# puzzlepaint/surfelmeshing

Measured on NVIDIA H100. Metric: RGB-D frames/s at 640x480 (depth pre-processing + Integrate()), higher is better.
Workload: dtype f32

## Files before the change

surfelmeshing_b200/csrc/integrate.cu:

```cuda

#include <algorithm>
#include <cstdio>
#include <cstdlib>

#include <cooperative_groups.h>

#include "sm_kernels.cuh"

namespace cg = cooperative_groups;

namespace smb {

namespace {

#define SM_S(row, i) d.surfels[static_cast<size_t>(row) * d.stride + (i)]
#define SM_SU(row, i) reinterpret_cast<u32*>(d.surfels)[static_cast<size_t>(row) * d.stride + (i)]

constexpr int kBlock = 256;

__device__ __forceinline__ bool is_active(u32 last_update_stamp, u32 frame_index, int window) {
  return static_cast<int>(last_update_stamp) > static_cast<int>(frame_index - static_cast<u32>(window));
}

struct Projection {
// ... 35 lines not shown
__device__ __forceinline__ float normal_z_abs(float nx, float ny) {
  return fsqrt_approx(fmaxf(0.f, ffma(-ny, ny, ffma(-nx, nx, 1.0f))));
}

__device__ __forceinline__ float facing_dot(const FrameParams& f, float x, float y, float z, float nx, float ny,
                                            float nz, float3* local_normal) {
  const float rs = frsqrt_approx(squared_norm(x, y, z));
  *local_normal = rotate_vec(f.local_T_global, nx, ny, nz);
  return fmul(rs, ffma(z, local_normal->z, ffma(x, local_normal->x, fmul(y, local_normal->y))));
}

template <typename Body>
__device__ __forceinline__ void for_each_visible(const DeviceState& d, const u32* surfel_count, Body&& body) {
  constexpr u32 kItemsPerSegment = kSegment / kBlock;
  const u32 max_items = ((d.capacity + kSegment - 1) / kSegment) * kItemsPerSegment;
  const u32 n = *surfel_count;
  u32 item = blockIdx.x;
  u32 cnt = 0;
  VisEntry e = make_uint4(0u, 0u, 0u, 0u);
  if (item < max_items) {
    cnt = d.seg_count[item / kItemsPerSegment];
    e = d.vis[static_cast<size_t>(item) * kBlock + threadIdx.x];
  }
  const u32 items = ((n + kSegment - 1) / kSegment) * kItemsPerSegment;
  while (item < items) {
    const u32 next = item + gridDim.x;
    u32 cnt_next = 0;
    VisEntry e_next = e;
    if (next < items) {
      cnt_next = d.seg_count[next / kItemsPerSegment];
      e_next = d.vis[static_cast<size_t>(next) * kBlock + threadIdx.x];
    }
    const u32 k = (item % kItemsPerSegment) * kBlock + threadIdx.x;
    if (k < cnt) body(static_cast<size_t>(item) * kBlock + threadIdx.x, e);
    item = next;
    cnt = cnt_next;
    e = e_next;
  }
}

__global__ void __launch_bounds__(kBlock) k_clear(DeviceState d) {
  pdl_prologue();
  const int n = d.width * d.height;
  for (int i = blockIdx.x * blockDim.x + threadIdx.x; i < n; i += gridDim.x * blockDim.x) {
    d.assoc[i] = make_uint4(kInvalidIndex, kInvalidIndex, 0u, 0u);
    d.first_depth[i] = __int_as_float(0x7f800000);
    d.supported[i] = 0;
  }
}

constexpr int kProjectBlock = 512;

enum { kProjectAll = 0, kProjectMain = 1, kProjectTail = 2 };

__global__ void __launch_bounds__(kProjectBlock) k_project(DeviceState d, FrameParams f, int part) {
  pdl_prologue();
  if (f.skip) return;
  const TimelineScope timeline_scope(d, f.frame_index, part == kProjectTail ? KID_PROJECT_TAIL : KID_PROJECT);
  __shared__ u32 warp_totals[kProjectBlock / 32];
  const int lane = threadIdx.x & 31, warp = threadIdx.x >> 5;
  const u32 first_seg_if_all = blockIdx.x;

  if (blockIdx.x == 0 && part != kProjectMain) {
    const int tiles = (d.width * d.height + kSegment - 1) / kSegment;
    for (int t = threadIdx.x; t < tiles; t += blockDim.x) d.scan_state[t] = 0ull;
    if (threadIdx.x == 0) { d.counters->scan_ticket = 0; *d.upd_count = 0; }
  }

  struct SlotRows { float2 X, Y, Z; uint2 T; };
  auto fetch = [&](u32 seg) {
    SlotRows r;
    const size_t base = static_cast<size_t>(seg) * kSegment + threadIdx.x * 2;
    r.X = *reinterpret_cast<const float2*>(&SM_S(SM_ROW_X, base));
    r.Y = *reinterpret_cast<const float2*>(&SM_S(SM_ROW_Y, base));
    r.Z = *reinterpret_cast<const float2*>(&SM_S(SM_ROW_Z, base));
    r.T = *reinterpret_cast<const uint2*>(&SM_SU(SM_ROW_LAST_UPDATE_STAMP, base));
    return r;
  };
  SlotRows rows = {};
  if (part != kProjectTail && (static_cast<size_t>(first_seg_if_all) + 1) * kSegment <= d.stride) rows = fetch(first_seg_if_all);
  const u32 n_before = part == kProjectAll ? 0u : d.counters->surfel_count[(f.count_slot + kCountSlots - 1) % kCountSlots];
  const u32 seg_begin = part == kProjectTail ? n_before / kSegment : 0u;
  const u32 n = part == kProjectMain ? (n_before / kSegment) * kSegment
                                     : d.counters->surfel_count[f.count_slot];
  if (part == kProjectTail && static_cast<u64>(seg_begin + blockIdx.x) * kSegment < n) rows = fetch(seg_begin + blockIdx.x);
  for (u32 seg = seg_begin + blockIdx.x; static_cast<u64>(seg) * kSegment < n; seg += gridDim.x) {
    const u32 base = seg * kSegment + threadIdx.x * 2;
    const SlotRows cur = rows;
    if (static_cast<u64>(seg + gridDim.x) * kSegment < n) rows = fetch(seg + gridDim.x);
    VisEntry e[2];
    bool visible[2] = {false, false};
    u32 cnt = 0;
    if (base < n) {
      const float xs[2] = {cur.X.x, cur.X.y}, ys[2] = {cur.Y.x, cur.Y.y}, zs[2] = {cur.Z.x, cur.Z.y};
      const u32 ts[2] = {cur.T.x, cur.T.y};
#pragma unroll
      for (int j = 0; j < 2; ++j) {
        const u32 i = base + j;
        if (i >= n) break;
        const float z = transform_row(f.local_T_global.r2, xs[j], ys[j], zs[j]);
        if (!(z > 0.f)) continue;
        const float x = transform_row(f.local_T_global.r0, xs[j], ys[j], zs[j]);
        const float y = transform_row(f.local_T_global.r1, xs[j], ys[j], zs[j]);
        const Projection p = project(f, d.width, d.height, x, y, z);
        if (!p.in_image) continue;
        const bool active = is_active(ts[j], f.frame_index, f.active_window);
        e[j] = make_uint4(i | (active ? kActiveBit : 0u), __float_as_uint(x), __float_as_uint(y), __float_as_uint(z));
        visible[j] = true;
        ++cnt;
        if (active) {
          atomicMin(reinterpret_cast<int*>(&d.first_depth[p.py * d.width + p.px]), __float_as_int(z));
          int ox, oy;
          if (secondary_pixel(p, d.width, d.height, &ox, &oy)) {
            atomicMin(reinterpret_cast<int*>(&d.first_depth[oy * d.width + ox]), __float_as_int(z));
          }
        }
      }
    }
    u32 incl = cnt;
#pragma unroll
// ... 87 lines not shown
      if (!pass[k]) continue;
      const PixelGate& g = k == 0 ? g0 : g1;
      const int pp = k == 0 ? p.py * d.width + p.px : oy * d.width + ox;
      if (!(g.measurement_depth > 0.f)) { pass[k] = false; continue; }
      if (g.first < fmul(g.measurement_depth, fadd(-f.sensor_noise_factor, 1.0f))) {
        if (g.first == z) d.assoc[pp].y = idx;
        pass[k] = false;
        continue;
      }
      if (z > fmul(fadd(f.sensor_noise_factor, 1.0f), g.measurement_depth)) pass[k] = false;
    }
    if (!pass[0] && !pass[1]) return;
    const float snx = SM_S(SM_ROW_NORMAL_X, idx), sny = SM_S(SM_ROW_NORMAL_Y, idx), snz = SM_S(SM_ROW_NORMAL_Z, idx);
    const float surfel_radius_squared = SM_S(SM_ROW_RADIUS_SQUARED, idx);
    g0.normal = row_ptr(f.normals, f.normals_pitch, pass[0] ? p.py : oy)[pass[0] ? p.px : ox];
    g1.normal = row_ptr(f.normals, f.normals_pitch, pass[1] ? oy : p.py)[pass[1] ? ox : p.px];
    float3 ln;
    const float dot_angle = facing_dot(f, x, y, z, snx, sny, snz, &ln);
#endif
#pragma unroll
    for (int k = 0; k < 2; ++k) {
      if (!pass[k]) continue;
      const int pp = k == 0 ? p.py * d.width + p.px : oy * d.width + ox;
#if SM_ASSOCIATE_LEVELS == 1
      if (!supports_surfel(d, f, k == 0 ? g0 : g1, pp, idx, z, dot_angle, ln)) continue;
#else
      {
        const PixelGate& g = k == 0 ? g0 : g1;
        if (dot_angle > 0.f) continue;
        if (g.measurement_depth < z) {
          const float s = normal_z_abs(g.normal.x, g.normal.y);
          const float dot2 = ffma(-ln.z, s, ffma(ln.x, g.normal.x, fmul(ln.y, g.normal.y)));
          if (dot2 < f.cos_normal_compatibility_threshold) continue;
        }
      }
#endif
      if (!(surfel_radius_squared > 0.f)) continue;
      PixelAssoc* a = &d.assoc[pp];
      atomicMin(&a->x, tb_encode(f.tb, idx, k == 1, static_cast<u32>(pp)));
      atomicAdd(&a->z, 1u);
      atomicAdd(reinterpret_cast<float*>(&a->w), z);
      d.supported[pp] = 1;
    }
  });
}

#ifndef SM_MERGE_LEVELS
#define SM_MERGE_LEVELS 2
#endif
__global__ void __launch_bounds__(kBlock) k_merge(DeviceState d, FrameParams f) {
  pdl_prologue();
  if (f.skip) return;
  const TimelineScope timeline_scope(d, f.frame_index, KID_MERGE);
  u32 merged_by_thread = 0;
#if SM_MERGE_LEVELS == 2
  for_each_visible(d, &d.counters->surfel_count[f.count_slot], [&](size_t pos, const VisEntry& e) {
    const u32 idx = e.x & ~kActiveBit;
    const float x = __uint_as_float(e.y), y = __uint_as_float(e.z), z = __uint_as_float(e.w);
    const Projection p = project(f, d.width, d.height, x, y, z);
    const int pp = p.py * d.width + p.px;
    const float surfel_radius_squared = SM_S(SM_ROW_RADIUS_SQUARED, idx);
    const float measurement_depth = fmul(u2f(row_ptr(f.depth_pre, f.depth_pre_pitch, p.py)[p.px]), f.inv_depth_scaling);
    const float first = d.first_depth[pp];
    const u32 supporting_key = d.assoc[pp].x;
    bool merged = false;
    if (surfel_radius_squared >= 0.f && measurement_depth > 0.f) {
      if (first < fmul(measurement_depth, fadd(-f.sensor_noise_factor, 1.0f))) {
        if (first == z) d.assoc[pp].y = idx;
      } else if (!(z > fmul(fadd(f.sensor_noise_factor, 1.0f), measurement_depth))) {
        const u32 q = supporting_index(f.tb, supporting_key, static_cast<u32>(pp));
        if (q != idx && q != kInvalidIndex) {
          const float snx = SM_S(SM_ROW_NORMAL_X, idx), sny = SM_S(SM_ROW_NORMAL_Y, idx), snz = SM_S(SM_ROW_NORMAL_Z, idx);
          const float gx = SM_S(SM_ROW_X, idx), gy = SM_S(SM_ROW_Y, idx), gz = SM_S(SM_ROW_Z, idx);
          const float2 pixel_normal = row_ptr(f.normals, f.normals_pitch, p.py)[p.px];
          const float other_radius_squared = SM_S(SM_ROW_RADIUS_SQUARED, q);
          const float qx = SM_S(SM_ROW_X, q), qy = SM_S(SM_ROW_Y, q), qz = SM_S(SM_ROW_Z, q);
          const float qnx = SM_S(SM_ROW_NORMAL_X, q), qny = SM_S(SM_ROW_NORMAL_Y, q), qnz = SM_S(SM_ROW_NORMAL_Z, q);
          float3 ln;
          const float dot_angle = facing_dot(f, x, y, z, snx, sny, snz, &ln);
          bool same_surface = !(dot_angle > 0.f);
          if (same_surface && measurement_depth < z) {
            const float s = normal_z_abs(pixel_normal.x, pixel_normal.y);
            const float dot2 = ffma(-ln.z, s, ffma(ln.x, pixel_normal.x, fmul(ln.y, pixel_normal.y)));
            same_surface = !(dot2 < f.cos_normal_compatibility_threshold);
          }
          if (same_surface) {
            const float radius_diff = fmul(surfel_radius_squared, frcp(other_radius_squared));
            const float distance_squared = squared_norm(fsub(gx, qx), fsub(gy, qy), fsub(gz, qz));
            merged = !(radius_diff > 1.4400000572204589844f || radius_diff < 0.69444441795349121094f) &&
                     !(distance_squared > fmul(fadd(surfel_radius_squared, other_radius_squared), 0.03125f)) &&
                     !(dot3(snx, sny, snz, qnx, qny, qnz) < 0.93968999385833740234f);
          }
        }
      }
    }
    d.merge_flag[pos] = merged ? 1 : 0;
    merged_by_thread += merged ? 1u : 0u;
  });
#else
  for_each_visible(d, &d.counters->surfel_count[f.count_slot], [&](size_t pos, const VisEntry& e) {
    const u32 idx = e.x & ~kActiveBit;
    const float x = __uint_as_float(e.y), y = __uint_as_float(e.z), z = __uint_as_float(e.w);
    const Projection p = project(f, d.width, d.height, x, y, z);
    const int pp = p.py * d.width + p.px;
    const PixelGate g = load_pixel_gate(d, f, p.px, p.py);
    const u32 supported_surfel = supporting_index(f.tb, d.assoc[pp].x, static_cast<u32>(pp));
// ... 828 lines not shown
    const float sz = fmul(fadd(g.z, sum_z), rcp_count);
    const float4 record = make_float4(sx, sy, sz, __uint_as_float(f.frame_index));
    d.smooth[idx] = record;
    d.smooth_next[idx] = record;
  }
}

__global__ void __launch_bounds__(kBlock) k_export_vertices(DeviceState d, int count_slot, float* position_buffer,
                                                            u8* color_buffer) {
  pdl_prologue();
  const u32 n = d.counters->surfel_count[count_slot];
  for (u32 i = blockIdx.x * blockDim.x + threadIdx.x; i < n; i += gridDim.x * blockDim.x) {
    const bool merged = SM_S(SM_ROW_RADIUS_SQUARED, i) < 0.f;
    const float nan = __int_as_float(0x7fffffff);
    const float4 smooth = d.smooth[i];
    position_buffer[3 * i + 0] = merged ? nan : smooth.x;
    position_buffer[3 * i + 1] = merged ? nan : smooth.y;
    position_buffer[3 * i + 2] = merged ? nan : smooth.z;
    const u32 c = SM_SU(SM_ROW_COLOR, i);
    color_buffer[3 * i + 0] = c & 0xFF;
    color_buffer[3 * i + 1] = (c >> 8) & 0xFF;
    color_buffer[3 * i + 2] = (c >> 16) & 0xFF;
  }
}

}

namespace {
size_t BlendSmemBytes(int radius) {
  const size_t rw = kBlendTileW + 2 * blend_halo_x(radius), rh = kBlendTileH + 2 * blend_halo_y(radius);
  const size_t rn16 = (rw * rh + 15) & ~static_cast<size_t>(15);
  const size_t mask_words = rh * ((rw + 31) / 32);
  return rn16 * 14 + mask_words * 11 * 4 + 16;
}
constexpr size_t kBlendSmemLimit = 224 * 1024;

#define SM_EV(call)                                                              \
  do {                                                                           \
    const cudaError_t e_ = (call);                                               \
    if (e_ != cudaSuccess) return SetError(SM_ERR_CUDA, cudaGetErrorString(e_)); \
  } while (0)
}

int DescribeFrameKernel(FrameKernel which, const LaunchPlan& plan, const DeviceState& d, const FrameParams& f,
                        KernelLaunch* out) {
  static_assert(sizeof(DeviceState) + sizeof(FrameParams) + 32 <= sizeof(out->storage), "KernelLaunch::storage too small");
  const int scan_tiles = (d.width * d.height + kSegment - 1) / kSegment;
  switch (which) {
    case FK_PROJECT:
    case FK_PROJECT_MAIN:
      out->Reset(reinterpret_cast<const void*>(k_project), dim3(plan.project), dim3(kProjectBlock), 0, KID_PROJECT);
      break;
    case FK_PROJECT_TAIL:
      out->Reset(reinterpret_cast<const void*>(k_project), dim3(plan.sm_count), dim3(kProjectBlock), 0, KID_PROJECT_TAIL);
      break;
    case FK_ASSOCIATE:
      out->Reset(reinterpret_cast<const void*>(k_associate), dim3(plan.associate), dim3(kBlock), 0, KID_ASSOCIATE);
      break;
    case FK_MERGE:
      out->Reset(reinterpret_cast<const void*>(k_merge), dim3(plan.merge), dim3(kBlock), 0, KID_MERGE);
      break;
    case FK_BLEND: {
      const size_t smem = BlendSmemBytes(f.blend_radius);
      if (f.blend_radius < 1 || f.blend_radius > kMaxBlendRadius || smem > kBlendSmemLimit)
        return SetError(SM_ERR_INVALID_ARGUMENT, "measurement_blending_radius too large for one tile region per SM");
      const dim3 pixel_tiles((d.width + kBlendTileW - 1) / kBlendTileW, (d.height + kBlendTileH - 1) / kBlendTileH);
      out->Reset(reinterpret_cast<const void*>(k_blend), pixel_tiles, dim3(kBlendBlock), smem, KID_BLEND);
      break;
    }
    case FK_INTEGRATE:
      out->Reset(reinterpret_cast<const void*>(k_integrate), dim3(plan.integrate), dim3(kBlock), 0, KID_INTEGRATE);
      break;
    case FK_UPDATE_NEIGHBORS:
      out->Reset(reinterpret_cast<const void*>(k_update_neighbors), dim3(plan.update_neighbors), dim3(kBlock), 0,
                 KID_UPDATE_NEIGHBORS);
      break;
    case FK_SCAN:
      out->Reset(reinterpret_cast<const void*>(k_new_surfel_scan), dim3(scan_tiles), dim3(kBlock), 0, KID_NEW_SURFEL_SCAN);
      break;
    case FK_CREATE:
      out->Reset(reinterpret_cast<const void*>(k_create_surfels), dim3(plan.sm_count * 2), dim3(kBlock), 0, KID_CREATE_SURFELS);
      break;
    default:
      return SetError(SM_ERR_INVALID_ARGUMENT, "DescribeFrameKernel");
  }
  out->Arg(d);
  out->Arg(f);
  if (which == FK_PROJECT) out->Arg(static_cast<int>(kProjectAll));
  if (which == FK_PROJECT_MAIN) out->Arg(static_cast<int>(kProjectMain));
  if (which == FK_PROJECT_TAIL) out->Arg(static_cast<int>(kProjectTail));
  return SM_OK;
}

namespace {
int LaunchFrameKernel(cudaStream_t stream, FrameKernel which, const LaunchPlan& plan, const DeviceState& d,
                      const FrameParams& f, bool dependent) {
  KernelLaunch k;
  const int status = DescribeFrameKernel(which, plan, d, f, &k);
  if (status != SM_OK) return status;
  LaunchOnStream(stream, k, dependent);
  return SM_OK;
}
}

int ClearAssociationRasters(cudaStream_t stream, const DeviceState& d) {
  const int blocks = (d.width * d.height + kBlock * 4 - 1) / (kBlock * 4);
  { LaunchScope scope(stream, KID_CLEAR); LaunchKernel(k_clear, dim3(blocks), dim3(kBlock), 0, stream, d); }
// ... 70 lines not shown
  } else {
    for (int i = 0; i < reg.iterations && status == SM_OK; ++i) {
      status = RegularizeSurfels(crit, d, false, f.frame_index, reg.radius_factor, reg.regularizer_weight, reg.window,
                                 new_slot, i == 0 ? old_slot : -1, plan);
    }
  }
  SM_EV(cudaEventRecord(pc->ev_reg, crit));
  pc->have_frame = true;
  return status;
}

int ExportVertices(cudaStream_t stream, const DeviceState& d, int count_slot, int sm_count, float* position_buffer,
                   u8* color_buffer) {
  { LaunchScope scope(stream, KID_EXPORT_VERTICES); LaunchKernel(k_export_vertices, dim3(sm_count * 8), dim3(kBlock), 0, stream, d, count_slot, position_buffer, color_buffer); }
  return CheckLaunch("export vertices");
}

int ConfigureIntegrateKernels(int carveout_percent, LaunchPlan* plan) {
  if (carveout_percent >= 0) {
    cudaFuncSetAttribute(k_clear, cudaFuncAttributePreferredSharedMemoryCarveout, carveout_percent);
    cudaFuncSetAttribute(k_project, cudaFuncAttributePreferredSharedMemoryCarveout, carveout_percent);
    cudaFuncSetAttribute(k_associate, cudaFuncAttributePreferredSharedMemoryCarveout, carveout_percent);
    cudaFuncSetAttribute(k_merge, cudaFuncAttributePreferredSharedMemoryCarveout, carveout_percent);
    cudaFuncSetAttribute(k_blend, cudaFuncAttributePreferredSharedMemoryCarveout, carveout_percent);
    cudaFuncSetAttribute(k_integrate, cudaFuncAttributePreferredSharedMemoryCarveout, carveout_percent);
    cudaFuncSetAttribute(k_update_neighbors, cudaFuncAttributePreferredSharedMemoryCarveout, carveout_percent);
    cudaFuncSetAttribute(k_new_surfel_scan, cudaFuncAttributePreferredSharedMemoryCarveout, carveout_percent);
    cudaFuncSetAttribute(k_create_surfels, cudaFuncAttributePreferredSharedMemoryCarveout, carveout_percent);
    cudaFuncSetAttribute(k_export_vertices, cudaFuncAttributePreferredSharedMemoryCarveout, carveout_percent);
    cudaGetLastError();
  }
  if (cudaFuncSetAttribute(k_blend, cudaFuncAttributeMaxDynamicSharedMemorySize, static_cast<int>(kBlendSmemLimit)) != cudaSuccess) {
    return SetError(SM_ERR_CUDA, "cudaFuncSetAttribute(k_blend, MaxDynamicSharedMemorySize)");
  }
  const int sm_count = plan->sm_count;
  const char* e = std::getenv("SM_B200_RESIDENT_GRIDS");
  if (e && e[0] == '0') {
    plan->project = sm_count * 4;
    plan->associate = plan->merge = plan->integrate = plan->update_neighbors = sm_count * 8;
    return SM_OK;
  }
  auto resident = [&](auto kernel, int block, int fallback_per_sm) {
    int per_sm = 0;
    if (cudaOccupancyMaxActiveBlocksPerMultiprocessor(&per_sm, kernel, block, 0) != cudaSuccess || per_sm < 1) {
      cudaGetLastError();
      per_sm = fallback_per_sm;
    }
    return ScaleGrid(sm_count * per_sm);
  };
  plan->project = resident(k_project, kProjectBlock, 2);
  plan->associate = resident(k_associate, kBlock, 8);
  plan->merge = resident(k_merge, kBlock, 4);
  plan->integrate = resident(k_integrate, kBlock, 3);
  plan->update_neighbors = resident(k_update_neighbors, kBlock, 3);
  if (const char* pe = std::getenv("SM_B200_OFFCHAIN_GRID_PERCENT")) {
    const int percent = std::atoi(pe);
    if (percent > 0 && percent < 100) {
      plan->update_neighbors = std::max(sm_count, plan->update_neighbors * percent / 100);
      plan->merge = std::max(sm_count, plan->merge * percent / 100);
    }
  }
  return SM_OK;
}

}
```

surfelmeshing_b200/csrc/pipeline.cu:

```cuda

#include <chrono>
#include <cstdio>
#include <cstdlib>
#include <string>

#include "sm_handle.cuh"

namespace smb {

namespace {

#define SM_CUDA(call)                                                                                   \
  do {                                                                                                  \
    const cudaError_t e_ = (call);                                                                      \
    if (e_ != cudaSuccess) return SetError(SM_ERR_CUDA, (std::string(#call) + ": " + cudaGetErrorString(e_)).c_str()); \
  } while (0)

constexpr int kDepthRing = 16;
constexpr int kColorRing = 6;
constexpr int kIterationEvents = 32;

int EnvInt(const char* name, int fallback) {
  const char* e = std::getenv(name);
  return (e && e[0]) ? std::atoi(e) : fallback;
// ... 228 lines not shown

  int status = SM_OK;
  if (c.first < c.last) {
    status = enqueue_preprocess(c.first);
    if (status != SM_OK) return status;
  }
  for (int frame = c.first; frame < c.last; ++frame) {
    const int set = frame & 1;
    if (frame + 1 < c.last) {
      status = enqueue_preprocess(frame + 1);
      if (status != SM_OK) return status;
    }
    SM_CUDA(cudaStreamWaitEvent(pipelined ? r->pipe.front : stream, r->pre_done[set], 0));
    r->d.assoc = r->assoc_set[set]; r->d.first_depth = r->first_depth_set[set]; r->d.supported = r->supported_set[set];
    r->d.vis = r->vis_set[set]; r->d.seg_count = r->seg_count_set[set]; r->d.merge_flag = r->merge_flag_set[set];
    r->d.upd_list = r->upd_list_set[set]; r->d.upd_count = r->upd_count_set[set];
    if (pipelined) {
      RecordOperation(r, static_cast<int>(static_cast<u32>(frame) - static_cast<u32>(c.ip->regularization_frame_window_size)));
      const FrameParams f = c.Params(frame, set);
      r->last_tiebreak = f.tb;
      RegularizeArgs reg;
      reg.iterations = c.ip->regularization_iterations_per_integration_iteration;
      reg.disable_denoising = reg.iterations == 0;
      reg.radius_factor = c.ip->radius_factor_for_regularization_neighbors;
      reg.regularizer_weight = c.ip->regularizer_weight;
      reg.window = c.ip->regularization_frame_window_size;
      status = IntegrateFramePipelined(r->pipe.front, &r->pipe, set, r->d, f, c.ip->do_blending != 0, reg, r->plan);
      if (status != SM_OK) return status;
      r->count_slot = (r->count_slot + 1) % kCountSlots;
    } else {
      r->rasters_cleared = true;
      size_t color_pitch;
      const uint8_t* color = c.Color(frame, &color_pitch);
      status = IntegrateImpl(r, stream, static_cast<u32>(frame), *c.ip, r->run_depth[set], r->run_depth_pitch,
                             reinterpret_cast<const float*>(r->run_normals[set]), r->run_normals_pitch,
                             r->run_radius[set], r->run_radius_pitch, color, color_pitch,
                             c.s->global_T_frame + 12 * frame, c.s->frame_T_global + 12 * frame);
      if (status != SM_OK) return status;
      SM_CUDA(cudaEventRecord(r->int_done[set], stream));
    }
    ++*integrated;
  }
  if (pipelined && r->pipe.have_frame) SM_CUDA(cudaStreamWaitEvent(stream, r->pipe.ev_reg, 0));
  return SM_OK;
}

}

struct FrameGraph {
  cudaGraph_t graph = nullptr;
  cudaGraphExec_t exec = nullptr;
  std::vector<cudaGraphNode_t> nodes;
  std::vector<const void*> funcs;
  int blending = -1, reg_launches = -1, pdl = -1, prio = -1, order = -1;
  size_t blend_smem = 0;
  dim3 scan_grid;
};

void DestroyFrameGraph(FrameGraph* g) {
  if (!g) return;
  if (g->exec) cudaGraphExecDestroy(g->exec);
  if (g->graph) cudaGraphDestroy(g->graph);
  delete g;
}

namespace {

struct StepLayout {
  int integrate, scan, update, create, reg0, reg_count, project, project_tail , associate,
      merge, blend , bilateral, tail, count;
};

StepLayout MakeLayout(bool blending, int reg_launches, bool split_project) {
  StepLayout l;
  int n = 0;
  l.integrate = n++; l.scan = n++; l.update = n++; l.create = n++;
  l.reg0 = n; l.reg_count = reg_launches; n += reg_launches;
  l.project = n++;
  l.project_tail = split_project ? n++ : -1;
  l.associate = n++; l.merge = n++;
  l.blend = blending ? n++ : -1;
  l.bilateral = n++; l.tail = n++;
  l.count = n;
  return l;
}

cudaKernelNodeParams NodeParams(const KernelLaunch& k) {
  cudaKernelNodeParams p = {};
  p.func = const_cast<void*>(k.func);
  p.gridDim = k.grid;
  p.blockDim = k.block;
  p.sharedMemBytes = static_cast<unsigned>(k.smem);
  p.kernelParams = const_cast<void**>(k.args);
  p.extra = nullptr;
  return p;
}

constexpr int kDefaultGraphOrder = 0;

int BuildFrameGraph(FrameGraph* g, const StepLayout& l, const std::vector<KernelLaunch>& launches, int pdl) {
  SM_CUDA(cudaGraphCreate(&g->graph, 0));
  g->nodes.assign(l.count, nullptr);
  g->funcs.assign(l.count, nullptr);
  for (int i = 0; i < l.count; ++i) {
    const cudaKernelNodeParams p = NodeParams(launches[i]);
    SM_CUDA(cudaGraphAddKernelNode(&g->nodes[i], g->graph, nullptr, 0, &p));
    g->funcs[i] = launches[i].func;
  }
  if (const int prio = EnvInt("SM_B200_GRAPH_PRIO", 0)) {
    int least = 0, greatest = 0;
    SM_CUDA(cudaDeviceGetStreamPriorityRange(&least, &greatest));
    auto set_priority = [&](int node, int priority) -> int {
      if (node < 0) return SM_OK;
      cudaKernelNodeAttrValue v = {};
      v.priority = priority;
      SM_CUDA(cudaGraphKernelNodeSetAttribute(g->nodes[node], cudaKernelNodeAttributePriority, &v));
      return SM_OK;
    };
    const int mid = (least + greatest) / 2;
    for (int i = 0; i < l.count; ++i) { const int st = set_priority(i, prio >= 2 ? mid : least); if (st != SM_OK) return st; }
    for (int node : {l.integrate, l.create, l.project, l.project_tail, l.associate, l.blend}) { const int st = set_priority(node, greatest); if (st != SM_OK) return st; }
    if (prio >= 2) for (int node : {l.bilateral, l.tail}) { const int st = set_priority(node, least); if (st != SM_OK) return st; }
  }
  std::vector<cudaGraphNode_t> from, to;
  std::vector<cudaGraphEdgeData> data;
  auto edge = [&](int a, int b, bool programmatic) {
    from.push_back(g->nodes[a]);
    to.push_back(g->nodes[b]);
    cudaGraphEdgeData e = {};
    if (pdl == 2 || (pdl == 1 && programmatic)) {
      e.from_port = cudaGraphKernelNodePortProgrammatic;
      e.type = cudaGraphDependencyTypeProgrammatic;
    }
    data.push_back(e);
  };
  edge(l.integrate, l.update, true);
  edge(l.integrate, l.create, false);
  edge(l.scan, l.create, false);
  if (l.reg_count > 0) {
    edge(l.update, l.reg0, false);
    edge(l.create, l.reg0, false);
    for (int i = 1; i < l.reg_count; ++i) edge(l.reg0 + i - 1, l.reg0 + i, true);
  }
  if (l.project_tail >= 0) {
    edge(l.integrate, l.project, false);
    edge(l.create, l.project_tail, false);
    edge(l.project, l.associate, false);
    edge(l.project_tail, l.associate, false);
  } else {
    edge(l.create, l.project, false);
    edge(l.project, l.associate, true);
  }
  edge(l.associate, l.merge, false);
  if (l.blend >= 0) edge(l.associate, l.blend, true);
  edge(l.bilateral, l.tail, true);
  const int order = EnvInt("SM_B200_GRAPH_ORDER", kDefaultGraphOrder);
  if (order & 1) edge(l.create, l.update, false);
  if ((order & 2) && l.reg_count > 0) edge(l.associate, l.reg0, false);
  if ((order & 4) && l.reg_count > 0) edge(l.merge, l.reg0, false);
  if (order & 8) edge(l.project_tail >= 0 ? l.project_tail : l.project, l.update, false);
  SM_CUDA(cudaGraphAddDependencies_v2(g->graph, from.data(), to.data(), data.data(), from.size()));
  SM_CUDA(cudaGraphInstantiate(&g->exec, g->graph, 0));
  return SM_OK;
}

int RunGraph(RunContext& c, cudaStream_t stream, uint32_t* integrated) {
  sm_reconstruction* r = c.r;
  const int W = c.W, H = c.H, half = c.half;
  const bool blending = c.ip->do_blending != 0;
  const int iterations = c.ip->regularization_iterations_per_integration_iteration;
  const bool disable_denoising = iterations == 0;
  const int reg_launches = disable_denoising ? 1 : 2 * iterations;
  const bool split_project = EnvInt("SM_B200_SPLIT_PROJECT", 0) != 0;
  const StepLayout l = MakeLayout(blending, reg_launches, split_project);
  const int pdl = EnvInt("SM_B200_GRAPH_PDL", 0);
  std::vector<KernelLaunch> launches(l.count);

  cudaStream_t gs = r->graph_stream;
  SM_CUDA(cudaEventRecord(r->entry_event, stream));
  SM_CUDA(cudaStreamWaitEvent(gs, r->entry_event, 0));
  if (c.depth_ring) SM_CUDA(cudaStreamWaitEvent(r->upload_stream, r->entry_event, 0));
  int uploaded_until = c.first - half - 1;
  const int it0 = c.first - 2;

  float4* smooth = r->d.smooth;
  float4* smooth_next = r->d.smooth_next;

  auto active = [&](int frame) { return frame >= c.first && frame < c.last; };
  auto clamp_frame = [&](int frame) { return frame < c.first ? c.first : (frame >= c.last ? c.last - 1 : frame); };

  for (int it = it0; it < c.last; ++it) {
    const int crit = it, front = it + 1, pre = it + 2;
    if (c.depth_ring && active(pre)) {
      for (int f = uploaded_until + 1; f <= pre + half; ++f) {
        const int last_reader_step = f - kDepthRing + half - 2;
        if (last_reader_step >= it0) SM_CUDA(cudaStreamWaitEvent(r->upload_stream, r->iteration_done[(last_reader_step - it0) % kIterationEvents], 0));
        const int st = c.EnqueueRawFrame(f);
        if (st != SM_OK) return st;
      }
      uploaded_until = pre + half;
      if (c.color_ring) {
        const int last_color_step = pre - kColorRing;
        if (last_color_step >= it0) SM_CUDA(cudaStreamWaitEvent(r->upload_stream, r->iteration_done[(last_color_step - it0) % kIterationEvents], 0));
        const int st = c.EnqueueColorFrame(pre);
        if (st != SM_OK) return st;
      }
      SM_CUDA(cudaEventRecord(r->upload_done, r->upload_stream));
      SM_CUDA(cudaStreamWaitEvent(gs, r->upload_done, 0));
    }

    int status = SM_OK;
    {
      const int frame = clamp_frame(crit), set = frame % kSets;
      DeviceState d = c.SetState(set);
      d.smooth = smooth; d.smooth_next = smooth_next;
      if (active(crit)) RecordOperation(r, static_cast<int>(static_cast<u32>(frame) - static_cast<u32>(c.ip->regularization_frame_window_size)));
      FrameParams f = c.Params(frame, set);
      f.skip = active(crit) ? 0 : 1;
      if (active(crit)) r->last_tiebreak = f.tb;
      const FrameKernel kernels[4] = {FK_INTEGRATE, FK_SCAN, FK_UPDATE_NEIGHBORS, FK_CREATE};
      const int slots[4] = {l.integrate, l.scan, l.update, l.create};
      for (int i = 0; i < 4; ++i) {
        status = DescribeFrameKernel(kernels[i], r->plan, d, f, &launches[slots[i]]);
        if (status != SM_OK) return status;
      }
      const int old_slot = f.count_slot, new_slot = (f.count_slot + 1) % kCountSlots;
      if (active(crit)) NoteIntegratedFrame(d, static_cast<u32>(frame));
      for (int i = 0; i < (disable_denoising ? 1 : iterations); ++i) {
        KernelLaunch* first = &launches[l.reg0 + (disable_denoising ? 0 : 2 * i)];
        KernelLaunch* second = disable_denoising ? nullptr : first + 1;
        DescribeRegularize(first, second, !active(crit), r->plan, d, disable_denoising, static_cast<u32>(frame),
                           c.ip->radius_factor_for_regularization_neighbors, c.ip->regularizer_weight,
                           c.ip->regularization_frame_window_size, new_slot, i == 0 ? old_slot : -1);
        if (!disable_denoising && active(crit)) {
          float4* const filled = smooth_next;
          smooth_next = smooth;
          smooth = filled;
          d.smooth = smooth; d.smooth_next = smooth_next;
          NoteRegStep(d, static_cast<u32>(frame), c.ip->regularization_frame_window_size);
        }
      }
      r->d.reg_t_prev = d.reg_t_prev;
      r->d.reg_full_sweep = d.reg_full_sweep;
      if (active(crit)) ++*integrated;
    }
    {
      const int frame = clamp_frame(front), set = frame % kSets;
      const DeviceState d = c.SetState(set);
      FrameParams f = c.Params(frame, set);
      f.skip = active(front) ? 0 : 1;
      const FrameKernel kernels[5] = {split_project ? FK_PROJECT_MAIN : FK_PROJECT, FK_PROJECT_TAIL, FK_ASSOCIATE, FK_MERGE, FK_BLEND};
      const int slots[5] = {l.project, l.project_tail, l.associate, l.merge, l.blend};
      for (int i = 0; i < 5; ++i) {
        if (slots[i] < 0) continue;
        status = DescribeFrameKernel(kernels[i], r->plan, d, f, &launches[slots[i]]);
        if (status != SM_OK) return status;
      }
    }
    {
      const int frame = clamp_frame(pre), set = frame % kSets;
      const u16* others[8];
      size_t other_pitches[8];
      c.Others(frame, others, other_pitches);
      size_t raw_pitch;
      const u16* raw = c.Raw(frame, &raw_pitch);
      status = DescribePreprocess(&launches[l.bilateral], &launches[l.tail], !active(pre), *c.pp, W, H, r->fx, r->fy,
                                  r->cx, r->cy, raw, raw_pitch, others, other_pitches,
                                  c.s->others_TR_reference + static_cast<size_t>(frame) * c.K * 12, r->scratch_B,
                                  r->scratch_B_pitch, r->run_depth[set], r->run_depth_pitch, r->run_normals[set],
                                  r->run_normals_pitch, r->run_radius[set], r->run_radius_pitch, r->assoc_set[set],
                                  r->first_depth_set[set], r->supported_set[set], r->run_depth_pre[set],
                                  r->run_depth_pitch, TimelineSlot(r->d, static_cast<u32>(frame), KID_BILATERAL_OUTLIER),
                                  TimelineSlot(r->d, static_cast<u32>(frame), KID_ERODE_NORMALS_RADII), r->ScratchBMap());
      if (status != SM_OK) return status;
    }

    FrameGraph* g = r->graph;
    const int prio = EnvInt("SM_B200_GRAPH_PRIO", 0);
    const int order = EnvInt("SM_B200_GRAPH_ORDER", kDefaultGraphOrder);
    bool rebuild = g == nullptr || g->blending != (blending ? 1 : 0) || g->reg_launches != reg_launches || g->pdl != pdl ||
                   g->prio != prio || g->order != order || static_cast<int>(g->nodes.size()) != l.count;
    if (!rebuild) {
      for (int i = 0; i < l.count && !rebuild; ++i) rebuild = g->funcs[i] != launches[i].func;
      if (l.blend >= 0) rebuild = rebuild || g->blend_smem != launches[l.blend].smem;
    }
    if (rebuild) {
      if (g) { SM_CUDA(cudaStreamSynchronize(gs)); DestroyFrameGraph(g); r->graph = nullptr; }
      g = new FrameGraph();
      r->graph = g;
      g->blending = blending ? 1 : 0; g->reg_launches = reg_launches; g->pdl = pdl; g->prio = prio; g->order = order;
      g->blend_smem = l.blend >= 0 ? launches[l.blend].smem : 0;
      status = BuildFrameGraph(g, l, launches, pdl);
      if (status != SM_OK) return status;
    } else {
      for (int i = 0; i < l.count; ++i) {
        const cudaKernelNodeParams p = NodeParams(launches[i]);
        SM_CUDA(cudaGraphExecKernelNodeSetParams(g->exec, g->nodes[i], &p));
      }
    }
    SM_CUDA(cudaGraphLaunch(g->exec, gs));
    CountLaunches(static_cast<unsigned long long>(l.count));
    if (c.depth_ring) SM_CUDA(cudaEventRecord(r->iteration_done[(it - it0) % kIterationEvents], gs));
  }
  r->d.smooth = smooth;
  r->d.smooth_next = smooth_next;
  {
    const DeviceState last_set = c.SetState((c.last - 1) % kSets);
    r->d.assoc = last_set.assoc; r->d.first_depth = last_set.first_depth; r->d.supported = last_set.supported;
    r->d.vis = last_set.vis; r->d.seg_count = last_set.seg_count; r->d.merge_flag = last_set.merge_flag;
    r->d.upd_list = last_set.upd_list; r->d.upd_count = last_set.upd_count;
  }
  r->count_slot = c.CountSlot(c.last);
  SM_CUDA(cudaEventRecord(r->graph_exit, gs));
  SM_CUDA(cudaStreamWaitEvent(stream, r->graph_exit, 0));
  return SM_OK;
}

}

int StreamRun(sm_reconstruction* r, cudaStream_t stream, const sm_stream_desc* s, const sm_preprocess_params* pp,
              const sm_integrate_params* ip, int first_frame, int last_frame, sm_stream_stats* stats) {
  RunContext c;
  c.r = r; c.s = s; c.pp = pp; c.ip = ip;
  c.W = r->d.width; c.H = r->d.height;
  c.pyramid = r->pyramid_level;
  if (c.pyramid > 0) {
    if (r->median_iterations > 0) {
      return SetError(SM_ERR_INVALID_ARGUMENT, "pyramid_level > 0 cannot be combined with median_filter_and_densify_iterations > 0");
    }
    const int step = 1 << c.pyramid;
    if (s->width <= 0 || s->height <= 0 || s->width % step != 0 || s->height % step != 0 ||
        (s->width >> c.pyramid) != c.W || (s->height >> c.pyramid) != c.H) {
      return SetError(SM_ERR_INVALID_ARGUMENT, "stream size must be the handle's size times 2^pyramid_level");
    }
  } else if (s->width != c.W || s->height != c.H) {
    return SetError(SM_ERR_INVALID_ARGUMENT, "stream size mismatch");
  }
  c.source_W = s->width; c.source_H = s->height;
  c.source_elems = static_cast<size_t>(c.source_W) * c.source_H;
  c.K = pp->outlier_filtering_frame_count;
  c.half = c.K / 2;
  if (c.K < 2 || c.K > 8 || first_frame < c.half || last_frame > s->frame_count - c.half || first_frame > last_frame) {
    return SetError(SM_ERR_INVALID_ARGUMENT,
                    "frame range needs outlier_filtering_frame_count/2 frames on both sides (main.cc:987-992)");
  }
// ... 40 lines not shown
```

surfelmeshing_b200/csrc/regularize.cu:

```cuda

#include <algorithm>
#include <cstdlib>

#include "sm_kernels.cuh"

namespace smb {

namespace {

#define SM_S(row, i) d.surfels[static_cast<size_t>(row) * d.stride + (i)]
#define SM_SU(row, i) reinterpret_cast<u32*>(d.surfels)[static_cast<size_t>(row) * d.stride + (i)]

constexpr int kBlock = 256;
#ifndef SM_REG_ACCUMULATE_MIN_BLOCKS
#define SM_REG_ACCUMULATE_MIN_BLOCKS 1
#endif
#ifndef SM_REG_STEP_MIN_BLOCKS
#define SM_REG_STEP_MIN_BLOCKS 1
#endif

struct RegParams {
  u32 frame_index;
  int window;
  float radius_factor_squared;
// ... 213 lines not shown
  p.skip = skip ? 1 : 0;
  p.t_prev = d.reg_t_prev;
  p.full_sweep = d.reg_full_sweep;
  static_assert(sizeof(DeviceState) + sizeof(RegParams) + 32 <= sizeof(first->storage), "KernelLaunch::storage too small");
  if (disable_denoising) {
    first->Reset(reinterpret_cast<const void*>(k_reg_copy_only), dim3(plan.reg_copy), dim3(kBlock), 0, KID_REG_COPY_ONLY);
    first->Arg(d);
    first->Arg(p);
    return 1;
  }
  first->Reset(reinterpret_cast<const void*>(k_reg_accumulate), dim3(plan.reg_accumulate), dim3(kBlock), 0, KID_REG_ACCUMULATE);
  first->Arg(d);
  first->Arg(p);
  second->Reset(reinterpret_cast<const void*>(k_reg_step), dim3(plan.reg_step), dim3(kBlock), 0, KID_REG_STEP);
  second->Arg(d);
  second->Arg(p);
  return 2;
}

int RegularizeSurfels(cudaStream_t stream, DeviceState& d, bool disable_denoising, u32 frame_index,
                      float radius_factor_for_regularization_neighbors, float regularizer_weight,
                      int regularization_frame_window_size, int count_slot, int remove_replaced_below_slot,
                      const LaunchPlan& plan) {
  KernelLaunch first, second;
  const int n = DescribeRegularize(&first, &second, false, plan, d, disable_denoising, frame_index,
                                   radius_factor_for_regularization_neighbors, regularizer_weight,
                                   regularization_frame_window_size, count_slot, remove_replaced_below_slot);
  LaunchOnStream(stream, first, false);
  if (n == 1) return CheckLaunch("regularize (copy only)");
  LaunchOnStream(stream, second, true);
  float4* const filled = d.smooth_next;
  d.smooth_next = d.smooth;
  d.smooth = filled;
  NoteRegStep(d, frame_index, regularization_frame_window_size);
  return CheckLaunch("regularize");
}

int ConfigureRegularizeKernels(int carveout_percent, LaunchPlan* plan) {
  if (carveout_percent >= 0) {
    cudaFuncSetAttribute(k_reg_accumulate, cudaFuncAttributePreferredSharedMemoryCarveout, carveout_percent);
    cudaFuncSetAttribute(k_reg_step, cudaFuncAttributePreferredSharedMemoryCarveout, carveout_percent);
    cudaFuncSetAttribute(k_reg_copy_only, cudaFuncAttributePreferredSharedMemoryCarveout, carveout_percent);
    cudaGetLastError();
  }
  const char* e = std::getenv("SM_B200_RESIDENT_GRIDS");
  auto resident = [&](auto kernel) {
    int per_sm = 0;
    if ((e && e[0] == '0') || cudaOccupancyMaxActiveBlocksPerMultiprocessor(&per_sm, kernel, kBlock, 0) != cudaSuccess || per_sm < 1) {
      cudaGetLastError();
      per_sm = 8;
    }
    return ScaleGrid(plan->sm_count * per_sm);
  };
  plan->reg_accumulate = resident(k_reg_accumulate);
  plan->reg_step = resident(k_reg_step);
  plan->reg_copy = resident(k_reg_copy_only);
  if (const char* pe = std::getenv("SM_B200_OFFCHAIN_GRID_PERCENT")) {
    const int percent = std::atoi(pe);
    if (percent > 0 && percent < 100) {
      plan->reg_accumulate = std::max(plan->sm_count, plan->reg_accumulate * percent / 100);
      plan->reg_step = std::max(plan->sm_count, plan->reg_step * percent / 100);
    }
  }
  return SM_OK;
}

}
```

surfelmeshing_b200/csrc/sm_kernels.cuh:

```cuda
#pragma once

#include <cuda_runtime.h>
#include <math.h>
#include <stddef.h>
#include <stdint.h>
#include <string.h>

#include "../../include/surfel_b200.h"
#include "sm_math.cuh"

namespace smb {

int SetError(int code, const char* message);
int CheckLaunch(const char* what);

enum KernelId {
  KID_CLEAR = 0, KID_BILATERAL_OUTLIER, KID_BILATERAL_GENERIC, KID_OUTLIER, KID_ERODE_NORMALS_RADII, KID_ERODE,
  KID_NORMALS, KID_RADII, KID_PROJECT, KID_ASSOCIATE, KID_MERGE, KID_BLEND, KID_INTEGRATE, KID_UPDATE_NEIGHBORS,
  KID_NEW_SURFEL_SCAN, KID_CREATE_SURFELS, KID_REG_ACCUMULATE, KID_REG_STEP, KID_REG_COPY_ONLY,
  KID_EXPORT_VERTICES, KID_MEDIAN_DENSIFY, KID_DELTA_SELECT, KID_VIZ_BUFFERS, KID_PROJECT_TAIL, KID_DOWNSCALE_DEPTH,
  KID_DOWNSCALE_COLOR, KID_REG_MIRROR, KID_REG_PACK, KID_COUNT
};
const char* KernelName(int id);
bool ProfilingEnabled();
// ... 202 lines not shown
                             cudaStream_t stream, Args&&... args) {
  cudaLaunchConfig_t cfg = {};
  cfg.gridDim = grid;
  cfg.blockDim = block;
  cfg.dynamicSmemBytes = smem;
  cfg.stream = stream;
  cudaLaunchAttribute attr[1];
  attr[0].id = cudaLaunchAttributeProgrammaticStreamSerialization;
  attr[0].val.programmaticStreamSerializationAllowed = 1;
  cfg.attrs = attr;
  const int mode = PdlMode();
  cfg.numAttrs = (mode == 2 || (mode == 1 && dependent)) ? 1 : 0;
  cudaLaunchKernelEx(&cfg, kernel, static_cast<KArgs>(args)...);
}
template <typename... KArgs, typename... Args>
inline void LaunchKernel(void (*kernel)(KArgs...), dim3 grid, dim3 block, size_t smem, cudaStream_t stream,
                         Args&&... args) {
  LaunchKernelImpl(false, kernel, grid, block, smem, stream, static_cast<Args&&>(args)...);
}
template <typename... KArgs, typename... Args>
inline void LaunchDependent(void (*kernel)(KArgs...), dim3 grid, dim3 block, size_t smem, cudaStream_t stream,
                            Args&&... args) {
  LaunchKernelImpl(true, kernel, grid, block, smem, stream, static_cast<Args&&>(args)...);
}

struct KernelLaunch {
  const void* func;
  dim3 grid, block;
  size_t smem;
  int kernel_id;
  int arg_count;
  void* args[4];
  alignas(64) unsigned char storage[2304];
  size_t used;
  void Reset(const void* f, dim3 g, dim3 b, size_t shared, int id) {
    func = f; grid = g; block = b; smem = shared; kernel_id = id; arg_count = 0; used = 0;
  }
  template <typename T>
  void Arg(const T& v) {
    used = (used + alignof(T) - 1) / alignof(T) * alignof(T);
    static_assert(alignof(T) <= 64, "argument alignment");
    memcpy(storage + used, &v, sizeof(T));
    args[arg_count++] = storage + used;
    used += sizeof(T);
  }
};
void LaunchOnStream(cudaStream_t stream, const KernelLaunch& k, bool dependent);

struct LaunchPlan {
  int sm_count;
  int project, associate, merge, integrate, update_neighbors;
  int reg_accumulate, reg_step, reg_copy;
};
int ConfigurePreprocessKernels(int carveout_percent);
int ConfigureIntegrateKernels(int carveout_percent, LaunchPlan* plan);
int ConfigureRegularizeKernels(int carveout_percent, LaunchPlan* plan);

struct alignas(64) TensorMapStorage { unsigned char bytes[128]; };
int MakeDepthTensorMap(TensorMapStorage* out, const u16* base, size_t pitch_bytes, int width, int height);
int PreprocessFused(cudaStream_t stream, const sm_preprocess_params& p, int width, int height, float fx, float fy,
                    float cx, float cy, const u16* raw, size_t raw_pitch, const u16* const* other_depths,
                    const size_t* other_pitches, const float* others_TR_reference, u16* scratch_B,
                    size_t scratch_B_pitch, u16* out_depth, size_t out_depth_pitch, float2* out_normals,
                    size_t out_normals_pitch, float* out_radius, size_t out_radius_pitch, uint4* clear_assoc,
                    float* clear_first_depth, u8* clear_supported, u16* out_depth_copy = nullptr,
                    size_t out_depth_copy_pitch = 0, unsigned long long* timeline_bilateral = nullptr,
                    unsigned long long* timeline_tail = nullptr, const TensorMapStorage* scratch_B_map = nullptr);
int DescribePreprocess(KernelLaunch* bilateral, KernelLaunch* tail, bool skip, const sm_preprocess_params& p, int width,
                       int height, float fx, float fy, float cx, float cy, const u16* raw, size_t raw_pitch,
                       const u16* const* other_depths, const size_t* other_pitches, const float* others_TR_reference,
                       u16* scratch_B, size_t scratch_B_pitch, u16* out_depth, size_t out_depth_pitch,
                       float2* out_normals, size_t out_normals_pitch, float* out_radius, size_t out_radius_pitch,
                       uint4* clear_assoc, float* clear_first_depth, u8* clear_supported, u16* out_depth_copy,
                       size_t out_depth_copy_pitch, unsigned long long* timeline_bilateral,
                       unsigned long long* timeline_tail, const TensorMapStorage* scratch_B_map);
int StageBilateral(cudaStream_t stream, float sigma_xy, float sigma_value_factor, u16 value_to_ignore,
                   float radius_factor, u16 max_depth, float depth_valid_region_radius, int width, int height,
                   const u16* in, size_t in_pitch, u16* out, size_t out_pitch);
int StageOutlier(cudaStream_t stream, int other_count, int required_count, float tolerance, float fx, float fy,
                 float cx, float cy, int width, int height, const u16* in, size_t in_pitch,
                 const u16* const* other_depths, const size_t* other_pitches, const float* others_TR_reference,
                 u16* out, size_t out_pitch);
int StageErode(cudaStream_t stream, int radius, int width, int height, const u16* in, size_t in_pitch, u16* out,
               size_t out_pitch);
int StageMedianDensify(cudaStream_t stream, int iterations, int width, int height, const u16* in, size_t in_pitch,
                       u16* out, size_t out_pitch, u16* scratch, size_t scratch_pitch);
int StageDownscaleMedian(cudaStream_t stream, u16 value_to_ignore, int in_width, int in_height, const u16* in,
                         size_t in_pitch, int out_width, int out_height, u16* out, size_t out_pitch);
int StageColorPyramid(cudaStream_t stream, int levels, int width, int height, const u8* in, size_t in_pitch, u8* out,
                      size_t out_pitch);
int StageNormals(cudaStream_t stream, float observation_angle_threshold_deg, float depth_scaling, float fx, float fy,
                 float cx, float cy, int width, int height, const u16* in, size_t in_pitch, u16* out, size_t out_pitch,
                 float2* normals, size_t normals_pitch);
int StageRadii(cudaStream_t stream, float point_radius_extension_factor, float point_radius_clamp_factor,
               float depth_scaling, float fx, float fy, float cx, float cy, int width, int height, const u16* in,
               size_t in_pitch, float* radius, size_t radius_pitch, u16* out, size_t out_pitch);

struct IntegrateEvents {
  cudaEvent_t ev[14];
  bool enabled;
};
int IntegrateFrame(cudaStream_t stream, const DeviceState& d, const FrameParams& f, bool do_blending,
                   bool rasters_already_cleared, const LaunchPlan& plan, const IntegrateEvents* events);
enum FrameKernel { FK_PROJECT = 0, FK_ASSOCIATE, FK_MERGE, FK_BLEND, FK_INTEGRATE, FK_UPDATE_NEIGHBORS, FK_SCAN, FK_CREATE,
                   FK_PROJECT_MAIN, FK_PROJECT_TAIL, FK_COUNT };
int DescribeFrameKernel(FrameKernel which, const LaunchPlan& plan, const DeviceState& d, const FrameParams& f,
// ... 43 lines not shown
```

Measured before the change: 9863.

## Make split project graph default, shrink off-chain grids, move scan reset to merge

Makes the split project (main plus tail) graph layout the default and removes the env-controlled PDL, priority and ordering options. The project tail now launches with 8 blocks instead of one per SM. The scan-state reset moves from the project tail into the merge kernel. Merge, update_neighbors and the regularization kernels now run with grids cut to 35% of their resident capacity. The aim is to let off-critical-path kernels overlap with the main chain inside the CUDA graph, at the cost of less parallelism for those kernels and a new ordering dependency for the scan reset.

```diff
diff --git a/surfelmeshing_b200/csrc/integrate.cu b/surfelmeshing_b200/csrc/integrate.cu
--- a/surfelmeshing_b200/csrc/integrate.cu
+++ b/surfelmeshing_b200/csrc/integrate.cu
@@ -111,6 +111,7 @@
 constexpr int kProjectBlock = 512;
 
 enum { kProjectAll = 0, kProjectMain = 1, kProjectTail = 2 };
+constexpr int kProjectTailBlocks = 8;
 
 __global__ void __launch_bounds__(kProjectBlock) k_project(DeviceState d, FrameParams f, int part) {
   pdl_prologue();
@@ -119,12 +120,6 @@
   __shared__ u32 warp_totals[kProjectBlock / 32];
   const int lane = threadIdx.x & 31, warp = threadIdx.x >> 5;
   const u32 first_seg_if_all = blockIdx.x;
-
-  if (blockIdx.x == 0 && part != kProjectMain) {
-    const int tiles = (d.width * d.height + kSegment - 1) / kSegment;
-    for (int t = threadIdx.x; t < tiles; t += blockDim.x) d.scan_state[t] = 0ull;
-    if (threadIdx.x == 0) { d.counters->scan_ticket = 0; *d.upd_count = 0; }
-  }
 
   struct SlotRows { float2 X, Y, Z; uint2 T; };
   auto fetch = [&](u32 seg) {
@@ -318,6 +313,11 @@
   pdl_prologue();
   if (f.skip) return;
   const TimelineScope timeline_scope(d, f.frame_index, KID_MERGE);
+  if (blockIdx.x == 0) {
+    const int tiles = (d.width * d.height + kSegment - 1) / kSegment;
+    for (int t = threadIdx.x; t < tiles; t += blockDim.x) d.scan_state[t] = 0ull;
+    if (threadIdx.x == 0) { d.counters->scan_ticket = 0; *d.upd_count = 0; }
+  }
   u32 merged_by_thread = 0;
 #if SM_MERGE_LEVELS == 2
   for_each_visible(d, &d.counters->surfel_count[f.count_slot], [&](size_t pos, const VisEntry& e) {
@@ -1252,7 +1252,7 @@
       out->Reset(reinterpret_cast<const void*>(k_project), dim3(plan.project), dim3(kProjectBlock), 0, KID_PROJECT);
       break;
     case FK_PROJECT_TAIL:
-      out->Reset(reinterpret_cast<const void*>(k_project), dim3(plan.sm_count), dim3(kProjectBlock), 0, KID_PROJECT_TAIL);
+      out->Reset(reinterpret_cast<const void*>(k_project), dim3(kProjectTailBlocks), dim3(kProjectBlock), 0, KID_PROJECT_TAIL);
       break;
     case FK_ASSOCIATE:
       out->Reset(reinterpret_cast<const void*>(k_associate), dim3(plan.associate), dim3(kBlock), 0, KID_ASSOCIATE);
@@ -1429,14 +1429,8 @@
   plan->associate = resident(k_associate, kBlock, 8);
   plan->merge = resident(k_merge, kBlock, 4);
   plan->integrate = resident(k_integrate, kBlock, 3);
-  plan->update_neighbors = resident(k_update_neighbors, kBlock, 3);
-  if (const char* pe = std::getenv("SM_B200_OFFCHAIN_GRID_PERCENT")) {
-    const int percent = std::atoi(pe);
-    if (percent > 0 && percent < 100) {
-      plan->update_neighbors = std::max(sm_count, plan->update_neighbors * percent / 100);
-      plan->merge = std::max(sm_count, plan->merge * percent / 100);
-    }
-  }
+  plan->update_neighbors = OffChainGrid(resident(k_update_neighbors, kBlock, 3), sm_count);
+  plan->merge = OffChainGrid(plan->merge, sm_count);
   return SM_OK;
 }
 
diff --git a/surfelmeshing_b200/csrc/pipeline.cu b/surfelmeshing_b200/csrc/pipeline.cu
--- a/surfelmeshing_b200/csrc/pipeline.cu
+++ b/surfelmeshing_b200/csrc/pipeline.cu
@@ -304,7 +304,7 @@
   cudaGraphExec_t exec = nullptr;
   std::vector<cudaGraphNode_t> nodes;
   std::vector<const void*> funcs;
-  int blending = -1, reg_launches = -1, pdl = -1, prio = -1, order = -1;
+  int blending = -1, reg_launches = -1;
   size_t blend_smem = 0;
   dim3 scan_grid;
 };
@@ -319,17 +319,17 @@
 namespace {
 
 struct StepLayout {
-  int integrate, scan, update, create, reg0, reg_count, project, project_tail , associate,
-      merge, blend , bilateral, tail, count;
+  int integrate, scan, update, create, reg0, reg_count, project, project_tail, associate, merge, blend ,
+      bilateral, tail, count;
 };
 
-StepLayout MakeLayout(bool blending, int reg_launches, bool split_project) {
+StepLayout MakeLayout(bool blending, int reg_launches) {
   StepLayout l;
   int n = 0;
   l.integrate = n++; l.scan = n++; l.update = n++; l.create = n++;
   l.reg0 = n; l.reg_count = reg_launches; n += reg_launches;
   l.project = n++;
-  l.project_tail = split_project ? n++ : -1;
+  l.project_tail = n++;
   l.associate = n++; l.merge = n++;
   l.blend = blending ? n++ : -1;
   l.bilateral = n++; l.tail = n++;
@@ -348,9 +348,7 @@
   return p;
 }
 
-constexpr int kDefaultGraphOrder = 0;
-
-int BuildFrameGraph(FrameGraph* g, const StepLayout& l, const std::vector<KernelLaunch>& launches, int pdl) {
+int BuildFrameGraph(FrameGraph* g, const StepLayout& l, const std::vector<KernelLaunch>& launches) {
   SM_CUDA(cudaGraphCreate(&g->graph, 0));
   g->nodes.assign(l.count, nullptr);
   g->funcs.assign(l.count, nullptr);
@@ -359,59 +357,27 @@
     SM_CUDA(cudaGraphAddKernelNode(&g->nodes[i], g->graph, nullptr, 0, &p));
     g->funcs[i] = launches[i].func;
   }
-  if (const int prio = EnvInt("SM_B200_GRAPH_PRIO", 0)) {
-    int least = 0, greatest = 0;
-    SM_CUDA(cudaDeviceGetStreamPriorityRange(&least, &greatest));
-    auto set_priority = [&](int node, int priority) -> int {
-      if (node < 0) return SM_OK;
-      cudaKernelNodeAttrValue v = {};
-      v.priority = priority;
-      SM_CUDA(cudaGraphKernelNodeSetAttribute(g->nodes[node], cudaKernelNodeAttributePriority, &v));
-      return SM_OK;
-    };
-    const int mid = (least + greatest) / 2;
-    for (int i = 0; i < l.count; ++i) { const int st = set_priority(i, prio >= 2 ? mid : least); if (st != SM_OK) return st; }
-    for (int node : {l.integrate, l.create, l.project, l.project_tail, l.associate, l.blend}) { const int st = set_priority(node, greatest); if (st != SM_OK) return st; }
-    if (prio >= 2) for (int node : {l.bilateral, l.tail}) { const int st = set_priority(node, least); if (st != SM_OK) return st; }
-  }
   std::vector<cudaGraphNode_t> from, to;
-  std::vector<cudaGraphEdgeData> data;
-  auto edge = [&](int a, int b, bool programmatic) {
+  auto edge = [&](int a, int b) {
     from.push_back(g->nodes[a]);
     to.push_back(g->nodes[b]);
-    cudaGraphEdgeData e = {};
-    if (pdl == 2 || (pdl == 1 && programmatic)) {
-      e.from_port = cudaGraphKernelNodePortProgrammatic;
-      e.type = cudaGraphDependencyTypeProgrammatic;
-    }
-    data.push_back(e);
   };
-  edge(l.integrate, l.update, true);
-  edge(l.integrate, l.create, false);
-  edge(l.scan, l.create, false);
+  edge(l.integrate, l.update);
+  edge(l.integrate, l.create);
+  edge(l.scan, l.create);
   if (l.reg_count > 0) {
-    edge(l.update, l.reg0, false);
-    edge(l.create, l.reg0, false);
-    for (int i = 1; i < l.reg_count; ++i) edge(l.reg0 + i - 1, l.reg0 + i, true);
-  }
-  if (l.project_tail >= 0) {
-    edge(l.integrate, l.project, false);
-    edge(l.create, l.project_tail, false);
-    edge(l.project, l.associate, false);
-    edge(l.project_tail, l.associate, false);
-  } else {
-    edge(l.create, l.project, false);
-    edge(l.project, l.associate, true);
-  }
-  edge(l.associate, l.merge, false);
-  if (l.blend >= 0) edge(l.associate, l.blend, true);
-  edge(l.bilateral, l.tail, true);
-  const int order = EnvInt("SM_B200_GRAPH_ORDER", kDefaultGraphOrder);
-  if (order & 1) edge(l.create, l.update, false);
-  if ((order & 2) && l.reg_count > 0) edge(l.associate, l.reg0, false);
-  if ((order & 4) && l.reg_count > 0) edge(l.merge, l.reg0, false);
-  if (order & 8) edge(l.project_tail >= 0 ? l.project_tail : l.project, l.update, false);
-  SM_CUDA(cudaGraphAddDependencies_v2(g->graph, from.data(), to.data(), data.data(), from.size()));
+    edge(l.update, l.reg0);
+    edge(l.create, l.reg0);
+    for (int i = 1; i < l.reg_count; ++i) edge(l.reg0 + i - 1, l.reg0 + i);
+  }
+  edge(l.integrate, l.project);
+  edge(l.create, l.project_tail);
+  edge(l.project, l.associate);
+  edge(l.project_tail, l.associate);
+  edge(l.associate, l.merge);
+  if (l.blend >= 0) edge(l.associate, l.blend);
+  edge(l.bilateral, l.tail);
+  SM_CUDA(cudaGraphAddDependencies(g->graph, from.data(), to.data(), from.size()));
   SM_CUDA(cudaGraphInstantiate(&g->exec, g->graph, 0));
   return SM_OK;
 }
@@ -423,9 +389,7 @@
   const int iterations = c.ip->regularization_iterations_per_integration_iteration;
   const bool disable_denoising = iterations == 0;
   const int reg_launches = disable_denoising ? 1 : 2 * iterations;
-  const bool split_project = EnvInt("SM_B200_SPLIT_PROJECT", 0) != 0;
-  const StepLayout l = MakeLayout(blending, reg_launches, split_project);
-  const int pdl = EnvInt("SM_B200_GRAPH_PDL", 0);
+  const StepLayout l = MakeLayout(blending, reg_launches);
   std::vector<KernelLaunch> launches(l.count);
 
   cudaStream_t gs = r->graph_stream;
@@ -501,7 +465,7 @@
       const DeviceState d = c.SetState(set);
       FrameParams f = c.Params(frame, set);
       f.skip = active(front) ? 0 : 1;
-      const FrameKernel kernels[5] = {split_project ? FK_PROJECT_MAIN : FK_PROJECT, FK_PROJECT_TAIL, FK_ASSOCIATE, FK_MERGE, FK_BLEND};
+      const FrameKernel kernels[5] = {FK_PROJECT_MAIN, FK_PROJECT_TAIL, FK_ASSOCIATE, FK_MERGE, FK_BLEND};
       const int slots[5] = {l.project, l.project_tail, l.associate, l.merge, l.blend};
       for (int i = 0; i < 5; ++i) {
         if (slots[i] < 0) continue;
@@ -528,10 +492,8 @@
     }
 
     FrameGraph* g = r->graph;
-    const int prio = EnvInt("SM_B200_GRAPH_PRIO", 0);
-    const int order = EnvInt("SM_B200_GRAPH_ORDER", kDefaultGraphOrder);
-    bool rebuild = g == nullptr || g->blending != (blending ? 1 : 0) || g->reg_launches != reg_launches || g->pdl != pdl ||
-                   g->prio != prio || g->order != order || static_cast<int>(g->nodes.size()) != l.count;
+    bool rebuild = g == nullptr || g->blending != (blending ? 1 : 0) || g->reg_launches != reg_launches ||
+                   static_cast<int>(g->nodes.size()) != l.count;
     if (!rebuild) {
       for (int i = 0; i < l.count && !rebuild; ++i) rebuild = g->funcs[i] != launches[i].func;
       if (l.blend >= 0) rebuild = rebuild || g->blend_smem != launches[l.blend].smem;
@@ -540,9 +502,9 @@
       if (g) { SM_CUDA(cudaStreamSynchronize(gs)); DestroyFrameGraph(g); r->graph = nullptr; }
       g = new FrameGraph();
       r->graph = g;
-      g->blending = blending ? 1 : 0; g->reg_launches = reg_launches; g->pdl = pdl; g->prio = prio; g->order = order;
+      g->blending = blending ? 1 : 0; g->reg_launches = reg_launches;
       g->blend_smem = l.blend >= 0 ? launches[l.blend].smem : 0;
-      status = BuildFrameGraph(g, l, launches, pdl);
+      status = BuildFrameGraph(g, l, launches);
       if (status != SM_OK) return status;
     } else {
       for (int i = 0; i < l.count; ++i) {
diff --git a/surfelmeshing_b200/csrc/regularize.cu b/surfelmeshing_b200/csrc/regularize.cu
--- a/surfelmeshing_b200/csrc/regularize.cu
+++ b/surfelmeshing_b200/csrc/regularize.cu
@@ -289,16 +289,9 @@
     }
     return ScaleGrid(plan->sm_count * per_sm);
   };
-  plan->reg_accumulate = resident(k_reg_accumulate);
-  plan->reg_step = resident(k_reg_step);
+  plan->reg_accumulate = OffChainGrid(resident(k_reg_accumulate), plan->sm_count);
+  plan->reg_step = OffChainGrid(resident(k_reg_step), plan->sm_count);
   plan->reg_copy = resident(k_reg_copy_only);
-  if (const char* pe = std::getenv("SM_B200_OFFCHAIN_GRID_PERCENT")) {
-    const int percent = std::atoi(pe);
-    if (percent > 0 && percent < 100) {
-      plan->reg_accumulate = std::max(plan->sm_count, plan->reg_accumulate * percent / 100);
-      plan->reg_step = std::max(plan->sm_count, plan->reg_step * percent / 100);
-    }
-  }
   return SM_OK;
 }
 
diff --git a/surfelmeshing_b200/csrc/sm_kernels.cuh b/surfelmeshing_b200/csrc/sm_kernels.cuh
--- a/surfelmeshing_b200/csrc/sm_kernels.cuh
+++ b/surfelmeshing_b200/csrc/sm_kernels.cuh
@@ -278,6 +278,10 @@
   int project, associate, merge, integrate, update_neighbors;
   int reg_accumulate, reg_step, reg_copy;
 };
+inline int OffChainGrid(int resident_blocks, int sm_count) {
+  const int blocks = resident_blocks * 35 / 100;
+  return blocks > sm_count ? blocks : sm_count;
+}
 int ConfigurePreprocessKernels(int carveout_percent);
 int ConfigureIntegrateKernels(int carveout_percent, LaunchPlan* plan);
 int ConfigureRegularizeKernels(int carveout_percent, LaunchPlan* plan);
```

New measurement: 10080, median of 6. +2.2%, better.
